# interaction-lab-uh/STROTSS-tensorflow

Measured on AMD Instinct MI355X. Metric: optimisation_steps_per_sec_1024px_pair, higher is better.
Workload: dtype f32; 1 GPU; 1024px content/style pair, 1024x1024 scale of the coarse-to-fine pyramid, 1024 samples x D=2179, VGG16 (seeded He-normal weights), RMSprop pixel update; scale_px=1024, samples=1024, parallelism=single GPU, tap_adjoint=deterministic (planned, sorted scatter)

## Files before the change

strotss-tensorflow_amd/csrc/image.hip:

```cpp
#include "internal.h"

namespace {

struct AxisTap { int lo, hi; float lerp; };
__device__ __forceinline__ AxisTap axis_tap(int i, float scale, int in_size) {
  const float src = __fsub_rn(__fmul_rn(__fadd_rn((float)i, 0.5f), scale), 0.5f);
  const float fl = floorf(src);
  AxisTap t;
  t.lo = max((int)fl, 0);
  t.hi = min((int)ceilf(src), in_size - 1);
  t.lerp = __fsub_rn(src, fl);
  return t;
}

template <int C>
__global__ __launch_bounds__(256) void resize_bilinear_kernel(const float* __restrict__ in, int ih, int iw,
                                                              int c_rt, float* __restrict__ out, int oh, int ow,
                                                              float sy, float sx, float alpha,
                                                              const float* __restrict__ add) {
  const int c = C ? C : c_rt;
  for (int oy = blockIdx.y; oy < oh; oy += gridDim.y) {
    const AxisTap ty = axis_tap(oy, sy, ih);
    const float* r0 = in + (size_t)ty.lo * iw * c;
    const float* r1 = in + (size_t)ty.hi * iw * c;
    const size_t orow = (size_t)oy * ow * c;
    for (int ox = blockIdx.x * 256 + threadIdx.x; ox < ow; ox += gridDim.x * 256) {
      const AxisTap tx = axis_tap(ox, sx, iw);
      const int a = tx.lo * c, b = tx.hi * c;
      const size_t o = orow + (size_t)ox * c;
#pragma unroll
      for (int ch = 0; ch < (C ? C : 1); ++ch)
        for (int cc = ch; cc < c; cc += (C ? C : 1)) {
          const float tl = r0[a + cc], tr = r0[b + cc], bl = r1[a + cc], br = r1[b + cc];
          const float top = tl + (tr - tl) * tx.lerp;
          const float bot = bl + (br - bl) * tx.lerp;
          float v = alpha * (top + (bot - top) * ty.lerp);
          if (add) v += add[o + cc];
          out[o + cc] = v;
        }
    }
  }
}

#define FOLD_TILE 32
#define FOLD_REGION 24
struct FoldLevels { int n; int h[STROTSS_MAX_TENSORS], w[STROTSS_MAX_TENSORS]; const float* v[STROTSS_MAX_TENSORS]; };
__device__ __forceinline__ float bilerp3(float tl, float tr, float bl, float br, float lx, float ly) {
  const float top = tl + (tr - tl) * lx;
  const float bot = bl + (br - bl) * lx;
  return 1.0f * (top + (bot - top) * ly);
}
__global__ __launch_bounds__(256) void fold_pyramid_kernel(FoldLevels p, float* __restrict__ img) {
  __shared__ float buf[2][FOLD_REGION * FOLD_REGION * 3];
  __shared__ int reg[STROTSS_MAX_TENSORS][4];
  const int t = threadIdx.x;
  if (t == 0) {
    int y0 = blockIdx.y * FOLD_TILE, y1 = min(y0 + FOLD_TILE, p.h[0]) - 1;
    int x0 = blockIdx.x * FOLD_TILE, x1 = min(x0 + FOLD_TILE, p.w[0]) - 1;
    reg[0][0] = y0; reg[0][1] = y1; reg[0][2] = x0; reg[0][3] = x1;
    for (int k = 1; k < p.n; ++k) {
      const float sy = (float)p.h[k] / (float)p.h[k - 1], sx = (float)p.w[k] / (float)p.w[k - 1];
      const int ny0 = axis_tap(y0, sy, p.h[k]).lo, ny1 = axis_tap(y1, sy, p.h[k]).hi;
      const int nx0 = axis_tap(x0, sx, p.w[k]).lo, nx1 = axis_tap(x1, sx, p.w[k]).hi;
      y0 = ny0; y1 = ny1; x0 = nx0; x1 = nx1;
      reg[k][0] = y0; reg[k][1] = y1; reg[k][2] = x0; reg[k][3] = x1;
    }
  }
  __syncthreads();
  {
    const int k = p.n - 1, y0 = reg[k][0], x0 = reg[k][2], rh = reg[k][1] - y0 + 1, rw = reg[k][3] - x0 + 1;
    float* dst = buf[k & 1];
    for (int e = t; e < rh * rw; e += 256) {
      const int ry = e / rw, rx = e - ry * rw;
      const float* s = p.v[k] + ((size_t)(y0 + ry) * p.w[k] + x0 + rx) * 3;
      dst[e * 3 + 0] = s[0]; dst[e * 3 + 1] = s[1]; dst[e * 3 + 2] = s[2];
    }
  }
  __syncthreads();
  for (int k = p.n - 2; k >= 0; --k) {
    const int y0 = reg[k][0], x0 = reg[k][2], rh = reg[k][1] - y0 + 1, rw = reg[k][3] - x0 + 1;
    const int cy0 = reg[k + 1][0], cx0 = reg[k + 1][2], cw = reg[k + 1][3] - cx0 + 1;
    const int ih = p.h[k + 1], iw = p.w[k + 1];
    const float sy = (float)ih / (float)p.h[k], sx = (float)iw / (float)p.w[k];
    const float* src = buf[(k + 1) & 1];
    float* dst = k == 0 ? nullptr : buf[k & 1];
    for (int e = t; e < rh * rw; e += 256) {
      const int ry = e / rw, rx = e - ry * rw;
      const int oy = y0 + ry, ox = x0 + rx;
      const AxisTap ty = axis_tap(oy, sy, ih), tx = axis_tap(ox, sx, iw);
      const float* r0 = src + (size_t)(ty.lo - cy0) * cw * 3;
      const float* r1 = src + (size_t)(ty.hi - cy0) * cw * 3;
      const int a = (tx.lo - cx0) * 3, b = (tx.hi - cx0) * 3;
      const size_t o = ((size_t)oy * p.w[k] + ox) * 3;
      const float* add = p.v[k] + o;
#pragma unroll
      for (int c = 0; c < 3; ++c) {
        float v = bilerp3(r0[a + c], r0[b + c], r1[a + c], r1[b + c], tx.lerp, ty.lerp);
        v += add[c];
        if (k == 0) img[o + c] = v; else dst[e * 3 + c] = v;
      }
    }
    __syncthreads();
  }
}

#define ADJ_MAX 8
__device__ __forceinline__ float adj_weight(int o, float scale, int in_size, int i) {
  const AxisTap t = axis_tap(o, scale, in_size);
  return (t.lo == i ? 1.0f - t.lerp : 0.f) + (t.hi == i ? t.lerp : 0.f);
}
struct AdjGlobal3 {
  const float* p; int ow;
  __device__ __forceinline__ const float* at(int oy, int ox) const { return p + ((size_t)oy * ow + ox) * 3; }
};
struct AdjRegion3 {
  const float* p; int y0, x0, rw;
  __device__ __forceinline__ const float* at(int oy, int ox) const { return p + ((oy - y0) * rw + (ox - x0)) * 3; }
};
__device__ __forceinline__ void adj_range(int i, float inv_scale, int out_size, int& o0, int& o1) {
  o0 = max(0, (int)floorf(((float)i - 0.5f) * inv_scale - 0.5f) - 1);
  o1 = min(out_size - 1, (int)ceilf(((float)i + 1.5f) * inv_scale - 0.5f) + 1);
}
template <class Src>
__device__ __forceinline__ void adjoint_pixel3(const Src& g, int oh, int ow, int ih, int iw, float sy, float sx, int iy,
                                               int ix, float (&acc)[3]) {
  int oy0, oy1, ox0, ox1;
  adj_range(iy, 1.0f / sy, oh, oy0, oy1);
  adj_range(ix, 1.0f / sx, ow, ox0, ox1);
  acc[0] = acc[1] = acc[2] = 0.f;
  if (ox1 - ox0 < ADJ_MAX) {
    float wx[ADJ_MAX];
#pragma unroll
    for (int q = 0; q < ADJ_MAX; ++q) wx[q] = (ox0 + q <= ox1) ? adj_weight(ox0 + q, sx, iw, ix) : 0.f;
    for (int oy = oy0; oy <= oy1; ++oy) {
      const float wy = adj_weight(oy, sy, ih, iy);
      if (wy == 0.f) continue;
      float row[3] = {0.f, 0.f, 0.f};
#pragma unroll
      for (int q = 0; q < ADJ_MAX; ++q)
        if (wx[q] != 0.f) {
          const float* p = g.at(oy, ox0 + q);
#pragma unroll
          for (int ch = 0; ch < 3; ++ch) row[ch] += wx[q] * p[ch];
        }
#pragma unroll
      for (int ch = 0; ch < 3; ++ch) acc[ch] += wy * row[ch];
    }
    return;
  }
  for (int oy = oy0; oy <= oy1; ++oy) {
    const float wy = adj_weight(oy, sy, ih, iy);
    if (wy == 0.f) continue;
    float row[3] = {0.f, 0.f, 0.f};
    for (int ox = ox0; ox <= ox1; ++ox) {
      const float w = adj_weight(ox, sx, iw, ix);
      if (w != 0.f) {
        const float* q = g.at(oy, ox);
#pragma unroll
        for (int ch = 0; ch < 3; ++ch) row[ch] += w * q[ch];
      }
    }
#pragma unroll
    for (int ch = 0; ch < 3; ++ch) acc[ch] += wy * row[ch];
  }
}

#define ADJ2_T2 8
#define ADJ2_REGION 32
__global__ __launch_bounds__(256) void resize_adjoint_pair_kernel(const float* __restrict__ g0, int h0, int w0,
                                                                  float* __restrict__ g1, int h1, int w1,
                                                                  float* __restrict__ g2, int h2, int w2) {
  __shared__ float mid[ADJ2_REGION * ADJ2_REGION * 3];
  const int t = threadIdx.x;
  const float sy1 = (float)h1 / (float)h0, sx1 = (float)w1 / (float)w0;
  const float sy2 = (float)h2 / (float)h1, sx2 = (float)w2 / (float)w1;
  const int ty0 = blockIdx.y * ADJ2_T2, ty1 = min(ty0 + ADJ2_T2, h2) - 1, tx0 = blockIdx.x * ADJ2_T2, tx1 = min(tx0 + ADJ2_T2, w2) - 1;
  const int oy0 = blockIdx.y * 2 * ADJ2_T2, oy1 = min(oy0 + 2 * ADJ2_T2, h1) - 1;
  const int ox0 = blockIdx.x * 2 * ADJ2_T2, ox1 = min(ox0 + 2 * ADJ2_T2, w1) - 1;
  const bool has2 = ty0 <= ty1 && tx0 <= tx1, own1 = oy0 <= oy1 && ox0 <= ox1;
  int ry0 = oy0, ry1 = oy1, rx0 = ox0, rx1 = ox1;
  if (has2) {
    int a, b, c, d;
    adj_range(ty0, 1.0f / sy2, h1, a, b); adj_range(ty1, 1.0f / sy2, h1, c, d);
    const int ny0 = a, ny1 = d;
    adj_range(tx0, 1.0f / sx2, w1, a, b); adj_range(tx1, 1.0f / sx2, w1, c, d);
    const int nx0 = a, nx1 = d;
    if (own1) { ry0 = min(ry0, ny0); ry1 = max(ry1, ny1); rx0 = min(rx0, nx0); rx1 = max(rx1, nx1); }
    else { ry0 = ny0; ry1 = ny1; rx0 = nx0; rx1 = nx1; }
  } else if (!own1) {
    return;
  }
  const int rh = ry1 - ry0 + 1, rw = rx1 - rx0 + 1;
  const AdjGlobal3 src0{g0, w0};
  for (int e = t; e < rh * rw; e += 256) {
    const int ry = e / rw, rx = e - ry * rw;
    const int iy = ry0 + ry, ix = rx0 + rx;
    float acc[3];
    adjoint_pixel3(src0, h0, w0, h1, w1, sy1, sx1, iy, ix, acc);
    mid[e * 3 + 0] = acc[0]; mid[e * 3 + 1] = acc[1]; mid[e * 3 + 2] = acc[2];
    if (own1 && iy >= oy0 && iy <= oy1 && ix >= ox0 && ix <= ox1) {
      float* o = g1 + ((size_t)iy * w1 + ix) * 3;
      o[0] = acc[0]; o[1] = acc[1]; o[2] = acc[2];
    }
  }
  __syncthreads();
  if (!has2) return;
  const AdjRegion3 src1{mid, ry0, rx0, rw};
  const int th = ty1 - ty0 + 1, tw = tx1 - tx0 + 1;
  for (int e = t; e < th * tw; e += 256) {
    const int iy = ty0 + e / tw, ix = tx0 + e % tw;
    float acc[3];
    adjoint_pixel3(src1, h1, w1, h2, w2, sy2, sx2, iy, ix, acc);
    float* o = g2 + ((size_t)iy * w2 + ix) * 3;
    o[0] = acc[0]; o[1] = acc[1]; o[2] = acc[2];
  }
}

template <int C>
__global__ __launch_bounds__(256) void resize_adjoint_kernel(const float* __restrict__ gout, int oh, int ow,
                                                             int c_rt, float* __restrict__ gin, int ih, int iw,
                                                             float sy, float sx) {
  const int c = C ? C : c_rt;
  const float isy = 1.0f / sy, isx = 1.0f / sx;
  for (int iy = blockIdx.y; iy < ih; iy += gridDim.y) {
    const int oy0 = max(0, (int)floorf(((float)iy - 0.5f) * isy - 0.5f) - 1);
    const int oy1 = min(oh - 1, (int)ceilf(((float)iy + 1.5f) * isy - 0.5f) + 1);
    for (int ix = blockIdx.x * 256 + threadIdx.x; ix < iw; ix += gridDim.x * 256) {
      const int ox0 = max(0, (int)floorf(((float)ix - 0.5f) * isx - 0.5f) - 1);
      const int ox1 = min(ow - 1, (int)ceilf(((float)ix + 1.5f) * isx - 0.5f) + 1);
      float acc[C ? C : 4];
#pragma unroll
      for (int ch = 0; ch < (C ? C : 4); ++ch) acc[ch] = 0.f;
      if (C && ox1 - ox0 < ADJ_MAX) {
        float wx[ADJ_MAX];
#pragma unroll
        for (int q = 0; q < ADJ_MAX; ++q) wx[q] = (ox0 + q <= ox1) ? adj_weight(ox0 + q, sx, iw, ix) : 0.f;
        for (int oy = oy0; oy <= oy1; ++oy) {
          const float wy = adj_weight(oy, sy, ih, iy);
          if (wy == 0.f) continue;
          const float* g = gout + ((size_t)oy * ow + ox0) * c;
          float row[C ? C : 1];
#pragma unroll
          for (int ch = 0; ch < C; ++ch) row[ch] = 0.f;
#pragma unroll
          for (int q = 0; q < ADJ_MAX; ++q)
            if (wx[q] != 0.f) {
#pragma unroll
              for (int ch = 0; ch < C; ++ch) row[ch] += wx[q] * g[q * c + ch];
            }
#pragma unroll
          for (int ch = 0; ch < C; ++ch) acc[ch] += wy * row[ch];
        }
#pragma unroll
        for (int ch = 0; ch < C; ++ch) gin[((size_t)iy * iw + ix) * c + ch] = acc[ch];
      } else {
        for (int ch0 = 0; ch0 < c; ch0 += 4) {
          const int nc = min(4, c - ch0);
          float a4[4] = {0.f, 0.f, 0.f, 0.f};
          for (int oy = oy0; oy <= oy1; ++oy) {
            const float wy = adj_weight(oy, sy, ih, iy);
            if (wy == 0.f) continue;
            float row[4] = {0.f, 0.f, 0.f, 0.f};
            for (int ox = ox0; ox <= ox1; ++ox) {
              const float w = adj_weight(ox, sx, iw, ix);
              if (w != 0.f)
                for (int ch = 0; ch < nc; ++ch) row[ch] += w * gout[((size_t)oy * ow + ox) * c + ch0 + ch];
            }
            for (int ch = 0; ch < nc; ++ch) a4[ch] += wy * row[ch];
          }
          for (int ch = 0; ch < nc; ++ch) gin[((size_t)iy * iw + ix) * c + ch0 + ch] = a4[ch];
        }
      }
    }
  }
}

struct SampleTap { int ia, ib, ic, id; float wa, wb, wc, wd; };

__device__ __forceinline__ SampleTap sample_tap(const strotss_maps_t& m, int k, float gx, float gy,
                                                int bilinear) {
  for (int q = 0; q < m.n_div[k]; ++q) {
    gx = __fdiv_rn(gx, m.div[q]);
    gy = __fdiv_rn(gy, m.div[q]);
  }
  const int h = m.h[k], w = m.w[k];
  SampleTap t;
  if (bilinear) {
    const float gxf = floorf(gx), gyf = floorf(gy);
    const float dx = gx - gxf, dy = gy - gyf;
    t.wa = (1.f - dx) * (1.f - dy);
    t.wb = (1.f - dx) * dy;
    t.wc = dx * (1.f - dy);
    t.wd = dx * dy;
    const int x0 = (int)fminf(fmaxf(gxf, 0.f), (float)(h - 1));
    const int y0 = (int)fminf(fmaxf(gyf, 0.f), (float)(w - 1));
    int x1 = min(x0 + 1, h - 1);
    const int y1 = min(y0 + 1, w - 1);
    int xa = x0;
    if (m.rows[k] > 0) {
      const int ra = x0 - m.row0[k], rb = x1 - m.row0[k];
      xa = min(max(ra, 0), m.rows[k] - 1);
      x1 = min(max(rb, 0), m.rows[k] - 1);
      if (m.window_drop & (int)(ra != xa)) { t.wa = 0.f; t.wb = 0.f; }
      if (m.window_drop & (int)(rb != x1)) { t.wc = 0.f; t.wd = 0.f; }
    }
    t.ia = xa * w + y0; t.ib = xa * w + y1; t.ic = x1 * w + y0; t.id = x1 * w + y1;
  } else {
    int xi = (int)fminf(fmaxf(gx, 0.f), (float)(h - 1));
    const int yi = (int)fminf(fmaxf(gy, 0.f), (float)(w - 1));
    if (m.rows[k] > 0) xi = min(max(xi - m.row0[k], 0), m.rows[k] - 1);
    t.ia = t.ib = t.ic = t.id = xi * w + yi;
    t.wa = 1.f; t.wb = t.wc = t.wd = 0.f;
  }
  return t;
}

__device__ __forceinline__ void gather_row(const strotss_maps_t& m, const float* __restrict__ idx, int s, int bilinear,
                                           float* __restrict__ out, int ld, int dtotal) {
  if (m.sample_range && (s < m.sample_range[0] || s >= m.sample_range[1])) return;
  const float gx = idx[2 * s], gy = idx[2 * s + 1];
  float* o = out + (size_t)s * ld;
  const int wave = __builtin_amdgcn_readfirstlane((int)threadIdx.x >> 6), lane = threadIdx.x & 63;
  int off = 0, chunk = 0;
  for (int k = 0; k < m.n_maps; ++k) {
    const int c = m.c[k], nchunk = (c + 63) >> 6;
    int q0 = (wave - chunk) & 3;
    if (q0 < nchunk) {
      const SampleTap t = sample_tap(m, k, gx, gy, bilinear);
      const float* src = m.map[k];
      if (bilinear) {
        const float* pa = src + (size_t)t.ia * c; const float* pb = src + (size_t)t.ib * c;
        const float* pc = src + (size_t)t.ic * c; const float* pd = src + (size_t)t.id * c;
        for (int q = q0; q < nchunk; q += 4) {
          const int ch = q * 64 + lane;
          if (ch < c) o[off + ch] = pa[ch] * t.wa + pb[ch] * t.wb + pc[ch] * t.wc + pd[ch] * t.wd;
        }
      } else {
        const float* pa = src + (size_t)t.ia * c;
        for (int q = q0; q < nchunk; q += 4) {
          const int ch = q * 64 + lane;
          if (ch < c) o[off + ch] = pa[ch];
        }
      }
    }
    off += c;
    chunk += nchunk;
  }
  for (int ch = dtotal + threadIdx.x; ch < ld; ch += 256) o[ch] = 0.f;
}
__global__ __launch_bounds__(256) void hypercol_gather_kernel(strotss_maps_t m, const float* __restrict__ idx,
                                                              int bilinear, float* __restrict__ out, int ld,
                                                              int dtotal) {
  gather_row(m, idx, blockIdx.x, bilinear, out, ld, dtotal);
}
__device__ __forceinline__ void gather2_body(const strotss_maps_t& ma, const strotss_maps_t& mb,
                                             const float* __restrict__ idx, int n, int bilinear, float* __restrict__ out_a,
                                             float* __restrict__ out_b, int ld, int dtotal_a, int dtotal_b,
                                             float* __restrict__ zero, int zero_rows, const int b) {
  if (b < n) {
    gather_row(ma, idx, b, bilinear, out_a, ld, dtotal_a);
    if (zero) {
      const int r1 = b == n - 1 ? zero_rows : min(b + 1, zero_rows);
      for (int r = b; r < r1; ++r)
        for (int ch = threadIdx.x; ch < ld; ch += 256) zero[(size_t)r * ld + ch] = 0.f;
    }
  } else {
    gather_row(mb, idx, b - n, bilinear, out_b, ld, dtotal_b);
  }
}
__global__ __launch_bounds__(256) void hypercol_gather2_kernel(strotss_maps_t ma, strotss_maps_t mb,
                                                               const float* __restrict__ idx, int n, int bilinear,
                                                               float* __restrict__ out_a, float* __restrict__ out_b, int ld,
                                                               int dtotal_a, int dtotal_b, float* __restrict__ zero,
                                                               int zero_rows) {
  gather2_body(ma, mb, idx, n, bilinear, out_a, out_b, ld, dtotal_a, dtotal_b, zero, zero_rows, (int)blockIdx.x);
}
__global__ __launch_bounds__(256) void hypercol_gather2_cw_kernel(strotss_maps_t ma, strotss_maps_t mb, strotss_maps_t mw,
                                                                  const float* __restrict__ idx, int n, int bilinear,
                                                                  float* __restrict__ out_a, float* __restrict__ out_b, int ld,
                                                                  int dtotal_a, int dtotal_b, float* __restrict__ zero,
                                                                  int zero_rows, float* __restrict__ wout, int wrows) {
  const int b = blockIdx.x;
  gather2_body(ma, mb, idx, n, bilinear, out_a, out_b, ld, dtotal_a, dtotal_b, zero, zero_rows, b);
  if (b < n) {
    gather_row(mw, idx, b, bilinear, wout, 1, 1);
    if (b == n - 1)
      for (int r = n + (int)threadIdx.x; r < wrows; r += 256) wout[r] = 0.f;
  }
}
#define SCATTER_DENSE_MAX_PIX 64
__device__ __forceinline__ void scatter_dense_block(const strotss_maps_t& m, const float* __restrict__ idx, int n,
                                                    const float* __restrict__ gfeat, int ld, bool masked, int k, int off, int b) {
  __shared__ int li[1024];
  __shared__ float lw[1024];
  __shared__ int cnts[4];
  __shared__ float red[4][64];
  const int tid = threadIdx.x, lane = tid & 63, wave = tid >> 6;
  const int c = m.c[k], nchunk = (c + 63) >> 6;
  const int p = b / nchunk, q = b - p * nchunk;
  const int s0 = m.sample_range ? m.sample_range[0] : 0, s1 = m.sample_range ? min(n, m.sample_range[1]) : n;
  const int ch = q * 64 + lane;
  const bool in = ch < c;
  const float* g = gfeat + off + (in ? ch : c - 1);
  float acc = 0.f;
  for (int base = s0; base < s1; base += 1024) {
    float w4[4];
    int cnt = 0;
#pragma unroll
    for (int u = 0; u < 4; ++u) {
      const int s = base + 4 * tid + u;
      float w = 0.f;
      if (s < s1) {
        const SampleTap t = sample_tap(m, k, idx[2 * s], idx[2 * s + 1], 1);
        w = (t.ia == p ? t.wa : 0.f) + (t.ib == p ? t.wb : 0.f) + (t.ic == p ? t.wc : 0.f) + (t.id == p ? t.wd : 0.f);
      }
      w4[u] = w;
      cnt += w != 0.f;
    }
    int incl = cnt;
#pragma unroll
    for (int o = 1; o < 64; o <<= 1) {
      const int up = __shfl_up(incl, o, 64);
      if (lane >= o) incl += up;
    }
    __syncthreads();
    if (lane == 63) cnts[wave] = incl;
    __syncthreads();
    int at = incl - cnt, total = 0;
#pragma unroll
    for (int wv = 0; wv < 4; ++wv) {
      at += wv < wave ? cnts[wv] : 0;
      total += cnts[wv];
    }
#pragma unroll
    for (int u = 0; u < 4; ++u)
      if (w4[u] != 0.f) { li[at] = base + 4 * tid + u; lw[at] = w4[u]; ++at; }
    __syncthreads();
    int e = wave;
    for (; e + 12 < total; e += 16) {
      float v[4];
#pragma unroll
      for (int u = 0; u < 4; ++u) v[u] = g[(size_t)li[e + 4 * u] * ld];
#pragma unroll
      for (int u = 0; u < 4; ++u) acc += lw[e + 4 * u] * v[u];
    }
    for (; e < total; e += 4) acc += lw[e] * g[(size_t)li[e] * ld];
  }
  red[wave][lane] = acc;
  __syncthreads();
  if (wave == 0 && in) {
    const float tot = (red[0][lane] + red[1][lane]) + (red[2][lane] + red[3][lane]);
    const size_t o = (size_t)p * c + ch;
    if (tot != 0.f && (!masked || m.map[k][o] > 0.f)) m.gmap[k][o] += tot;
  }
}
__global__ __launch_bounds__(256) void hypercol_scatter_kernel(strotss_maps_t m, const float* __restrict__ idx,
                                                               const float* __restrict__ gfeat, int ld,
                                                               int relu_mask_from, int map_begin,
                                                               int map_end, int n, unsigned dense_mask, int dense_blocks) {
  if ((int)blockIdx.x < dense_blocks) {
    int b = (int)blockIdx.x, off = 0;
    for (int k = 0; k < map_end; ++k) {
      if ((dense_mask >> k) & 1u) {
        const int nb = (m.rows[k] > 0 ? m.rows[k] : m.h[k]) * m.w[k] * ((m.c[k] + 63) >> 6);
        if (b < nb) { scatter_dense_block(m, idx, n, gfeat, ld, k >= relu_mask_from, k, off, b); return; }
        b -= nb;
      }
      off += m.c[k];
    }
    return;
  }
  const int s = (int)blockIdx.x - dense_blocks;
  if (m.sample_range && (s < m.sample_range[0] || s >= m.sample_range[1])) return;
  const float gx = idx[2 * s], gy = idx[2 * s + 1];
  const float* g = gfeat + (size_t)s * ld;
  const int wave = __builtin_amdgcn_readfirstlane((int)threadIdx.x >> 6), lane = threadIdx.x & 63;
  int off = 0, chunk = 0;
  for (int k = 0; k < map_end; ++k) {
    const int c = m.c[k], nchunk = (c + 63) >> 6;
    const int q0 = (wave - chunk) & 3;
    chunk += nchunk;
    if (k < map_begin || q0 >= nchunk || ((dense_mask >> k) & 1u)) { off += c; continue; }
    const SampleTap t = sample_tap(m, k, gx, gy, 1);
    const float* act = m.map[k];
    float* dst = m.gmap[k];
    const bool masked = k >= relu_mask_from;
    const int ii[4] = {t.ia, t.ib, t.ic, t.id};
    const float ww[4] = {t.wa, t.wb, t.wc, t.wd};
    for (int q = q0; q < nchunk; q += 4) {
      const int ch = q * 64 + lane;
      const bool in = ch < c;
      const int chc = in ? ch : c - 1;
      const float gv = in ? g[off + chc] : 0.f;
#pragma unroll
      for (int tq = 0; tq < 4; ++tq) {
        const float v = ww[tq] * gv;
        const size_t o = (size_t)ii[tq] * c + chc;
        if (v != 0.f && (!masked || act[o] > 0.f)) atomicAdd(&dst[o], v);
      }
    }
    off += c;
  }
}

#define PLAN_E 4096
struct PlanView {
  int* nseg; int* seg_start; int* pix; int* smp; float* w;
  __host__ __device__ static size_t ints_per_map() { return 2 + (PLAN_E + 1) + 3 * (size_t)PLAN_E + 1; }
  __host__ __device__ PlanView(void* base, int k) {
    int* b = reinterpret_cast<int*>(base) + (size_t)k * ints_per_map();
    nseg = b; seg_start = b + 2; pix = seg_start + PLAN_E + 1; smp = pix + PLAN_E; w = reinterpret_cast<float*>(smp + PLAN_E);
  }
};
__global__ __launch_bounds__(1024) void scatter_plan_kernel(strotss_maps_t m, const float* __restrict__ idx, int n,
                                                            void* __restrict__ plan) {
  __shared__ unsigned long long key[PLAN_E];
  __shared__ int wsum[16];
  const int k = blockIdx.x, t = threadIdx.x;
  const unsigned long long INVALID = ~0ull;
  const int s_begin = m.sample_range ? m.sample_range[0] : 0, s_end = m.sample_range ? min(n, m.sample_range[1]) : n;
  for (int e = t; e < PLAN_E; e += 1024) {
    const int s = e >> 2, q = e & 3;
    unsigned long long kk = INVALID;
    if (s >= s_begin && s < s_end) {
      const SampleTap tp = sample_tap(m, k, idx[2 * s], idx[2 * s + 1], 1);
      const int ii = q == 0 ? tp.ia : q == 1 ? tp.ib : q == 2 ? tp.ic : tp.id;
      const float ww = q == 0 ? tp.wa : q == 1 ? tp.wb : q == 2 ? tp.wc : tp.wd;
      if (ww != 0.f) kk = ((unsigned long long)(unsigned)ii << 12) | (unsigned)e;
    }
    key[e] = kk;
  }
  __syncthreads();
  for (int size = 2; size <= PLAN_E; size <<= 1)
    for (int stride = size >> 1; stride > 0; stride >>= 1) {
      for (int p = t; p < PLAN_E / 2; p += 1024) {
        const int lo = 2 * p - (p & (stride - 1));
        const int hi = lo + stride;
        const bool up = (lo & size) == 0;
        const unsigned long long a = key[lo], b = key[hi];
        if ((a > b) == up) { key[lo] = b; key[hi] = a; }
      }
      __syncthreads();
    }
  PlanView pv(plan, k);
  int head[4], cnt = 0, valid = 0;
#pragma unroll
  for (int i = 0; i < 4; ++i) {
    const int p = 4 * t + i;
    const unsigned long long a = key[p];
    const bool ok = a != INVALID;
    head[i] = ok && (p == 0 || (key[p - 1] >> 12) != (a >> 12));
    cnt += head[i]; valid += ok;
  }
  int incl = cnt, vincl = valid;
#pragma unroll
  for (int o = 1; o < 64; o <<= 1) {
    const int u = __shfl_up(incl, o, 64), v = __shfl_up(vincl, o, 64);
    if ((t & 63) >= o) { incl += u; vincl += v; }
  }
  if ((t & 63) == 63) { wsum[t >> 6] = incl; }
  __syncthreads();
  int base = incl - cnt;
  for (int wv = 0; wv < (t >> 6); ++wv) base += wsum[wv];
  int total = 0;
#pragma unroll
  for (int wv = 0; wv < 16; ++wv) total += wsum[wv];
  __syncthreads();
  if ((t & 63) == 63) wsum[t >> 6] = vincl;
  __syncthreads();
  int nvalid = 0;
#pragma unroll
  for (int wv = 0; wv < 16; ++wv) nvalid += wsum[wv];
#pragma unroll
  for (int i = 0; i < 4; ++i) {
    const int p = 4 * t + i;
    const unsigned long long a = key[p];
    if (a == INVALID) continue;
    const int e = (int)(a & 4095u), s = e >> 2, q = e & 3;
    const SampleTap tp = sample_tap(m, k, idx[2 * s], idx[2 * s + 1], 1);
    pv.pix[p] = (int)(a >> 12);
    pv.smp[p] = s;
    pv.w[p] = q == 0 ? tp.wa : q == 1 ? tp.wb : q == 2 ? tp.wc : tp.wd;
    if (head[i]) pv.seg_start[base++] = p;
  }
  if (t == 0) { pv.nseg[0] = total; pv.seg_start[total] = nvalid; }
}
__global__ __launch_bounds__(256) void scatter_sorted_kernel(strotss_maps_t m, int k, int off, const void* __restrict__ plan,
                                                             const float* __restrict__ gfeat, int ld, int masked) {
  PlanView pv(const_cast<void*>(plan), k);
  const int sg = blockIdx.x;
  if (sg >= pv.nseg[0]) return;
  const int p0 = pv.seg_start[sg], p1 = pv.seg_start[sg + 1];
  const int c = m.c[k];
  const size_t pixel = (size_t)pv.pix[p0] * c;
  const float* act = m.map[k];
  float* dst = m.gmap[k];
  for (int ch = threadIdx.x; ch < c; ch += 256) {
    if (masked && !(act[pixel + ch] > 0.f)) continue;
    float acc = 0.f;
    for (int p = p0; p < p1; ++p) acc += pv.w[p] * gfeat[(size_t)pv.smp[p] * ld + off + ch];
    dst[pixel + ch] += acc;
  }
}

__global__ __launch_bounds__(256) void rmsprop_kernel(strotss_tensors_t t, float lr, float rho, float eps) {
  const int k = blockIdx.y;
  float* var = t.var[k];
  float* rms = t.rms[k];
  const float* g = t.grad[k];
  const int64_t n = t.numel[k];
  const float omr = 1.0f - rho;
  for (int64_t e = (int64_t)blockIdx.x * 256 + threadIdx.x; e < n; e += (int64_t)gridDim.x * 256) {
    const float gv = g[e];
    const float r = rho * rms[e] + omr * (gv * gv);
    rms[e] = r;
    var[e] = var[e] - lr * gv / (sqrtf(r) + eps);
  }
}

__global__ __launch_bounds__(256) void minmax_partial_kernel(const float* __restrict__ x, int64_t n,
                                                             float* __restrict__ ws) {
  __shared__ float red[4];
  float mn = INFINITY, mx = -INFINITY;
  for (int64_t e = (int64_t)blockIdx.x * 256 + threadIdx.x; e < n; e += (int64_t)gridDim.x * 256) {
    const float v = fminf(fmaxf(x[e], 0.f), 1.f);
    mn = fminf(mn, v);
    mx = fmaxf(mx, v);
  }
  mn = block_min_256(mn, red);
  mx = block_max_256(mx, red);
  if (threadIdx.x == 0) { ws[blockIdx.x] = mn; ws[1024 + blockIdx.x] = mx; }
}
__global__ __launch_bounds__(256) void postprocess_kernel(const float* __restrict__ x, int64_t n,
                                                          const float* __restrict__ ws, int nparts,
                                                          uint8_t* __restrict__ out) {
  __shared__ float red[4];
  float mn = INFINITY, mx = -INFINITY;
  for (int i = threadIdx.x; i < nparts; i += 256) { mn = fminf(mn, ws[i]); mx = fmaxf(mx, ws[1024 + i]); }
  mn = block_min_256(mn, red);
  mx = block_max_256(mx, red);
  const float range = mx - mn;
  for (int64_t e = (int64_t)blockIdx.x * 256 + threadIdx.x; e < n; e += (int64_t)gridDim.x * 256) {
    float v = fminf(fmaxf(x[e], 0.f), 1.f);
    v = (v - mn) / range;
    out[e] = (uint8_t)(v * 255.0f);
  }
}

int maps_ok(const strotss_maps_t* m) {
  if (!m || m->n_maps <= 0 || m->n_maps > STROTSS_MAX_MAPS) return 0;
  for (int k = 0; k < m->n_maps; ++k) {
    if (m->h[k] <= 0 || m->w[k] <= 0 || m->c[k] <= 0 || !m->map[k]) return 0;
    if (m->n_div[k] < 0 || m->n_div[k] > STROTSS_MAX_DIVS) return 0;
    if (m->rows[k] < 0 || m->row0[k] < 0 || m->row0[k] + m->rows[k] > m->h[k]) return 0;
  }
  return 1;
}

}

extern "C" {

int strotss_abi_version(void) { return 8; }
const char* strotss_build_info(void) { return "libstrotss_hip gfx950 fp32-mfma " __DATE__ " " __TIME__; }

int strotss_resize_bilinear(const float* in, int ih, int iw, int c, float* out, int oh, int ow, float alpha,
                            const float* add, void* stream) {
  ST_CHECK_ARG(in && out && ih > 0 && iw > 0 && oh > 0 && ow > 0 && c > 0, STROTSS_EINVAL);
  const float sy = (float)ih / (float)oh, sx = (float)iw / (float)ow;
  const dim3 grid((unsigned)cdiv(ow, 256), (unsigned)min(oh, 32768));
  if (c == 3)
    hipLaunchKernelGGL(resize_bilinear_kernel<3>, grid, dim3(256), 0, (hipStream_t)stream, in, ih, iw, c, out, oh, ow, sy, sx,
                       alpha, add);
  else if (c == 1)
    hipLaunchKernelGGL(resize_bilinear_kernel<1>, grid, dim3(256), 0, (hipStream_t)stream, in, ih, iw, c, out, oh, ow, sy, sx,
                       alpha, add);
  else
    hipLaunchKernelGGL(resize_bilinear_kernel<0>, grid, dim3(256), 0, (hipStream_t)stream, in, ih, iw, c, out, oh, ow, sy, sx,
                       alpha, add);
  ST_LAUNCH_RET();
}

int strotss_fold_pyramid(const strotss_pyramid_t* pyr, float* img, void* stream) {
  ST_CHECK_ARG(pyr && img && pyr->n_levels >= 2 && pyr->n_levels <= STROTSS_MAX_TENSORS, STROTSS_EINVAL);
  FoldLevels p;
  p.n = pyr->n_levels;
  for (int k = 0; k < p.n; ++k) {
    ST_CHECK_ARG(pyr->var[k] && pyr->h[k] > 0 && pyr->w[k] > 0, STROTSS_EINVAL);
    p.h[k] = pyr->h[k]; p.w[k] = pyr->w[k]; p.v[k] = pyr->var[k];
  }
  int sy = FOLD_TILE, sx = FOLD_TILE;
  for (int k = 1; k < p.n; ++k) {
    ST_CHECK_ARG(p.h[k] <= p.h[k - 1] && p.w[k] <= p.w[k - 1], STROTSS_ERANGE);
    sy = min(p.h[k], (int)((long long)sy * p.h[k] / p.h[k - 1]) + 3);
    sx = min(p.w[k], (int)((long long)sx * p.w[k] / p.w[k - 1]) + 3);
    ST_CHECK_ARG(sy <= FOLD_REGION && sx <= FOLD_REGION, STROTSS_ERANGE);
  }
  hipLaunchKernelGGL(fold_pyramid_kernel, dim3((unsigned)cdiv(p.w[0], FOLD_TILE), (unsigned)cdiv(p.h[0], FOLD_TILE)), dim3(256),
                     0, (hipStream_t)stream, p, img);
  ST_LAUNCH_RET();
}

static bool adjoint_pair_ok(int a, int b) { return b >= 1 && a >= 2 * b - 1 && a <= 2 * b + 1; }

int strotss_fold_pyramid_adjoint(const strotss_pyramid_t* g, void* stream) {
  ST_CHECK_ARG(g && g->n_levels >= 2 && g->n_levels <= STROTSS_MAX_TENSORS, STROTSS_EINVAL);
  for (int k = 0; k < g->n_levels; ++k) ST_CHECK_ARG(g->var[k] && g->h[k] > 0 && g->w[k] > 0, STROTSS_EINVAL);
  int k = 0;
  while (k + 1 < g->n_levels) {
    const bool pair = k + 2 < g->n_levels && adjoint_pair_ok(g->h[k], g->h[k + 1]) && adjoint_pair_ok(g->w[k], g->w[k + 1]) &&
                      adjoint_pair_ok(g->h[k + 1], g->h[k + 2]) && adjoint_pair_ok(g->w[k + 1], g->w[k + 2]);
    if (pair) {
      const unsigned gx = (unsigned)max(cdiv(g->w[k + 2], ADJ2_T2), cdiv(g->w[k + 1], 2 * ADJ2_T2));
      const unsigned gy = (unsigned)max(cdiv(g->h[k + 2], ADJ2_T2), cdiv(g->h[k + 1], 2 * ADJ2_T2));
      hipLaunchKernelGGL(resize_adjoint_pair_kernel, dim3(gx, gy), dim3(256), 0, (hipStream_t)stream,
                         (const float*)g->var[k], g->h[k], g->w[k], const_cast<float*>(g->var[k + 1]), g->h[k + 1], g->w[k + 1],
                         const_cast<float*>(g->var[k + 2]), g->h[k + 2], g->w[k + 2]);
      k += 2;
    } else {
      const int rc = strotss_resize_bilinear_adjoint(g->var[k], g->h[k], g->w[k], 3, const_cast<float*>(g->var[k + 1]),
                                                     g->h[k + 1], g->w[k + 1], stream);
      if (rc != 0) return rc;
      k += 1;
    }
  }
  ST_LAUNCH_RET();
}

int strotss_resize_bilinear_adjoint(const float* gout, int oh, int ow, int c, float* gin, int ih, int iw,
                                    void* stream) {
  ST_CHECK_ARG(gout && gin && ih > 0 && iw > 0 && oh > 0 && ow > 0 && c > 0, STROTSS_EINVAL);
  const float sy = (float)ih / (float)oh, sx = (float)iw / (float)ow;
  const dim3 grid((unsigned)cdiv(iw, 256), (unsigned)min(ih, 32768));
  if (c == 3)
    hipLaunchKernelGGL(resize_adjoint_kernel<3>, grid, dim3(256), 0, (hipStream_t)stream, gout, oh, ow, c, gin, ih, iw, sy, sx);
  else if (c == 1)
    hipLaunchKernelGGL(resize_adjoint_kernel<1>, grid, dim3(256), 0, (hipStream_t)stream, gout, oh, ow, c, gin, ih, iw, sy, sx);
  else
    hipLaunchKernelGGL(resize_adjoint_kernel<0>, grid, dim3(256), 0, (hipStream_t)stream, gout, oh, ow, c, gin, ih, iw, sy, sx);
  ST_LAUNCH_RET();
}

int strotss_hypercol_gather(const strotss_maps_t* maps, const float* idx, int n, int bilinear, float* out,
                            int ld, void* stream) {
  ST_CHECK_ARG(maps_ok(maps) && idx && out && n > 0, STROTSS_EINVAL);
  int d = 0;
  for (int k = 0; k < maps->n_maps; ++k) d += maps->c[k];
  ST_CHECK_ARG(ld >= d, STROTSS_EINVAL);
  strotss_maps_t m = *maps;
  m.window_drop = 0;
  hipLaunchKernelGGL(hypercol_gather_kernel, dim3(n), dim3(256), 0, (hipStream_t)stream, m, idx, bilinear,
                     out, ld, d);
  ST_LAUNCH_RET();
}

int strotss_hypercol_gather2(const strotss_maps_t* maps_a, const strotss_maps_t* maps_b, const float* idx, int n,
                             int bilinear, float* out_a, float* out_b, int ld, float* zero, int zero_rows, void* stream) {
  ST_CHECK_ARG(maps_ok(maps_a) && maps_ok(maps_b) && idx && out_a && out_b && n > 0, STROTSS_EINVAL);
  ST_CHECK_ARG(!zero || zero_rows > 0, STROTSS_EINVAL);
  int da = 0, db = 0;
  for (int k = 0; k < maps_a->n_maps; ++k) da += maps_a->c[k];
  for (int k = 0; k < maps_b->n_maps; ++k) db += maps_b->c[k];
  ST_CHECK_ARG(ld >= da && ld >= db, STROTSS_EINVAL);
  strotss_maps_t a = *maps_a, b = *maps_b;
  a.window_drop = b.window_drop = 0;
  hipLaunchKernelGGL(hypercol_gather2_kernel, dim3(2 * n), dim3(256), 0, (hipStream_t)stream, a, b, idx, n, bilinear, out_a,
                     out_b, ld, da, db, zero, zero_rows);
  ST_LAUNCH_RET();
}

int strotss_hypercol_gather2_cw(const strotss_maps_t* maps_a, const strotss_maps_t* maps_b, const strotss_maps_t* maps_w,
                                const float* idx, int n, int bilinear, float* out_a, float* out_b, int ld, float* zero,
                                int zero_rows, float* weight_out, int weight_rows, void* stream) {
  ST_CHECK_ARG(maps_ok(maps_a) && maps_ok(maps_b) && maps_ok(maps_w) && idx && out_a && out_b && weight_out && n > 0,
               STROTSS_EINVAL);
  ST_CHECK_ARG(maps_w->n_maps == 1 && maps_w->c[0] == 1 && maps_w->rows[0] == 0 && weight_rows >= n, STROTSS_EINVAL);
  ST_CHECK_ARG(!zero || zero_rows > 0, STROTSS_EINVAL);
  int da = 0, db = 0;
  for (int k = 0; k < maps_a->n_maps; ++k) da += maps_a->c[k];
  for (int k = 0; k < maps_b->n_maps; ++k) db += maps_b->c[k];
  ST_CHECK_ARG(ld >= da && ld >= db, STROTSS_EINVAL);
  strotss_maps_t a = *maps_a, b = *maps_b, wm = *maps_w;
  a.window_drop = b.window_drop = wm.window_drop = 0;
  wm.sample_range = nullptr;
  hipLaunchKernelGGL(hypercol_gather2_cw_kernel, dim3(2 * n), dim3(256), 0, (hipStream_t)stream, a, b, wm, idx, n, bilinear,
                     out_a, out_b, ld, da, db, zero, zero_rows, weight_out, weight_rows);
  ST_LAUNCH_RET();
}

int strotss_hypercol_scatter(const strotss_maps_t* maps, const float* idx, int n, const float* gfeat, int ld,
                             int relu_mask_from, int map_begin, int map_end, void* stream) {
  ST_CHECK_ARG(maps_ok(maps) && idx && gfeat && n > 0, STROTSS_EINVAL);
  ST_CHECK_ARG(map_begin >= 0 && map_begin < map_end && map_end <= maps->n_maps, STROTSS_ERANGE);
  int d = 0;
  for (int k = 0; k < maps->n_maps; ++k) {
    if (k >= map_begin && k < map_end) ST_CHECK_ARG(maps->gmap[k] != nullptr, STROTSS_EINVAL);
    d += maps->c[k];
  }
  ST_CHECK_ARG(ld >= d, STROTSS_EINVAL);
  static const int dense_pix = [] {
    const char* e = getenv("STROTSS_SCATTER_DENSE");
    const int v = e ? atoi(e) : 1;
    return v == 1 ? SCATTER_DENSE_MAX_PIX : v;
  }();
  unsigned dense_mask = 0;
  int dense_blocks = 0;
  for (int k = map_begin; k < map_end; ++k) {
    const int pix = (maps->rows[k] > 0 ? maps->rows[k] : maps->h[k]) * maps->w[k];
    if (pix <= dense_pix) { dense_mask |= 1u << k; dense_blocks += pix * ((maps->c[k] + 63) / 64); }
  }
  hipLaunchKernelGGL(hypercol_scatter_kernel, dim3(n + dense_blocks), dim3(256), 0, (hipStream_t)stream, *maps, idx, gfeat,
                     ld, relu_mask_from, map_begin, map_end, n, dense_mask, dense_blocks);
  ST_LAUNCH_RET();
}

size_t strotss_hypercol_scatter_plan_bytes(int n_maps) {
  return n_maps > 0 ? (size_t)n_maps * PlanView::ints_per_map() * sizeof(int) : 0;
}

int strotss_hypercol_scatter_plan(const strotss_maps_t* maps, const float* idx, int n, void* plan, size_t plan_bytes,
                                  void* stream) {
  ST_CHECK_ARG(maps_ok(maps) && idx && plan && n > 0, STROTSS_EINVAL);
  ST_CHECK_ARG(4 * n <= PLAN_E, STROTSS_ERANGE);
  ST_CHECK_ARG(plan_bytes >= strotss_hypercol_scatter_plan_bytes(maps->n_maps), STROTSS_EINVAL);
  for (int k = 0; k < maps->n_maps; ++k) {
    const long long px = (long long)(maps->rows[k] > 0 ? maps->rows[k] : maps->h[k]) * maps->w[k];
    ST_CHECK_ARG(px < (1ll << 31), STROTSS_ERANGE);
  }
  hipLaunchKernelGGL(scatter_plan_kernel, dim3(maps->n_maps), dim3(1024), 0, (hipStream_t)stream, *maps, idx, n, plan);
  ST_LAUNCH_RET();
}

int strotss_hypercol_scatter_sorted(const strotss_maps_t* maps, const void* plan, int n, const float* gfeat, int ld,
                                    int relu_mask_from, int map_begin, int map_end, void* stream) {
  ST_CHECK_ARG(maps_ok(maps) && plan && gfeat && n > 0 && 4 * n <= PLAN_E, STROTSS_EINVAL);
  ST_CHECK_ARG(map_begin >= 0 && map_begin < map_end && map_end <= maps->n_maps, STROTSS_ERANGE);
  int off = 0;
  for (int k = 0; k < map_end; ++k) {
    if (k >= map_begin) {
      ST_CHECK_ARG(maps->gmap[k] != nullptr && off + maps->c[k] <= ld, STROTSS_EINVAL);
      hipLaunchKernelGGL(scatter_sorted_kernel, dim3(4 * n), dim3(256), 0, (hipStream_t)stream, *maps, k, off, plan, gfeat,
                         ld, k >= relu_mask_from ? 1 : 0);
    }
    off += maps->c[k];
  }
  ST_LAUNCH_RET();
}

int strotss_rmsprop_step(const strotss_tensors_t* t, float lr, float rho, float eps, void* stream) {
  ST_CHECK_ARG(t && t->n_tensors > 0 && t->n_tensors <= STROTSS_MAX_TENSORS, STROTSS_ERANGE);
  int64_t mx = 0;
  for (int k = 0; k < t->n_tensors; ++k) {
    ST_CHECK_ARG(t->var[k] && t->rms[k] && t->grad[k] && t->numel[k] > 0, STROTSS_EINVAL);
    mx = t->numel[k] > mx ? t->numel[k] : mx;
  }
  dim3 grid((unsigned)((mx + 255) / 256 > 2048 ? 2048 : (mx + 255) / 256), t->n_tensors);
  hipLaunchKernelGGL(rmsprop_kernel, grid, dim3(256), 0, (hipStream_t)stream, *t, lr, rho, eps);
  ST_LAUNCH_RET();
}

int strotss_postprocess(const float* img, int64_t numel, uint8_t* out, float* workspace, void* stream) {
  ST_CHECK_ARG(img && out && workspace && numel > 0, STROTSS_EINVAL);
  const int nparts = (int)((numel + 255) / 256 > 1024 ? 1024 : (numel + 255) / 256);
  hipLaunchKernelGGL(minmax_partial_kernel, dim3(nparts), dim3(256), 0, (hipStream_t)stream, img, numel,
                     workspace);
  hipLaunchKernelGGL(postprocess_kernel, dim3(nparts), dim3(256), 0, (hipStream_t)stream, img, numel,
                     workspace, nparts, out);
  ST_LAUNCH_RET();
}

}
```

strotss-tensorflow_amd/csrc/sort_match.h:

```cpp
#pragma once
#include "common.h"

namespace {

constexpr int SORT_T = 1024;

__device__ __forceinline__ unsigned long long ordered_pack(float v, int idx) {
  unsigned b = __float_as_uint(v);
  if (b == 0x80000000u) b = 0u;
  const unsigned key = (b & 0x80000000u) ? ~b : (b | 0x80000000u);
  return ((unsigned long long)key << 32) | (unsigned)idx;
}
__device__ __forceinline__ float ordered_value(unsigned long long c) {
  const unsigned key = (unsigned)(c >> 32);
  return __uint_as_float((key & 0x80000000u) ? (key & 0x7FFFFFFFu) : ~key);
}

template <int SIDES>
__device__ __forceinline__ void bitonic_sort_1024(unsigned long long (&v)[SIDES], unsigned long long* buf0,
                                                  unsigned long long* buf1, int S) {
  const int tid = threadIdx.x;
  int cross = 0;
#pragma unroll
  for (int k = 2; k <= SORT_T; k <<= 1) {
#pragma unroll
    for (int j = k >> 1; j > 0; j >>= 1) {
      unsigned long long* const buf = (cross & 1) ? buf1 : buf0;
      if (j >= 64) ++cross;
      if (k > S) continue;
      unsigned long long pv[SIDES];
      if (j < 64) {
#pragma unroll
        for (int s = 0; s < SIDES; ++s)
          pv[s] = ((unsigned long long)__shfl_xor((unsigned)(v[s] >> 32), j, 64) << 32) | __shfl_xor((unsigned)v[s], j, 64);
      } else {
#pragma unroll
        for (int s = 0; s < SIDES; ++s) buf[s * SORT_T + tid] = v[s];
        __syncthreads();
#pragma unroll
        for (int s = 0; s < SIDES; ++s) pv[s] = buf[s * SORT_T + (tid ^ j)];
      }
      const bool keep_low = ((tid & j) == 0) == ((tid & k) == 0);
#pragma unroll
      for (int s = 0; s < SIDES; ++s) v[s] = (v[s] < pv[s]) == keep_low ? v[s] : pv[s];
    }
  }
}

struct SquaredCost {
  static __device__ __forceinline__ void pair(float len, float diff, float& g, float& w) {
    g += len * diff;
    w += len * diff * diff;
  }
};
struct AbsoluteCost {
  static __device__ __forceinline__ void pair(float len, float diff, float& g, float& w) {
    g += diff > 0.f ? len : (diff < 0.f ? -len : 0.f);
    w += len * fabsf(diff);
  }
};

struct QuantileMatch {
  float coef;
  int row;
  float cost;
};

template <class Cost>
__device__ __forceinline__ QuantileMatch quantile_match(unsigned long long va, unsigned long long vb, int n, int ns,
                                                        float* sb) {
  const int tid = threadIdx.x;
  if (tid < ns) sb[tid] = ordered_value(vb);
  __syncthreads();
  QuantileMatch m = {0.f, 0, 0.f};
  if (tid < n) {
    const float a = ordered_value(va);
    const int lo = tid * ns, hi = lo + ns;
    float g = 0.f, w = 0.f;
    for (int j = lo / n; j < ns && j * n < hi; ++j) {
      const float len = (float)(min(hi, (j + 1) * n) - max(lo, j * n));
      const float diff = a - sb[j];
      Cost::pair(len, diff, g, w);
    }
    const float inv = (float)(1.0 / ((double)n * ns));
    m.coef = g * inv;
    m.row = (int)(unsigned)(va & 0xFFFFFFFFull);
    m.cost = w * inv;
  }
  return m;
}

__device__ __forceinline__ double block_sum_f64_1024(double v, double* red) {
  const int tid = threadIdx.x;
  v = wave_sum(v);
  if ((tid & 63) == 0) red[tid >> 6] = v;
  __syncthreads();
  double s = 0.0;
  if (tid == 0) {
#pragma unroll
    for (int i = 0; i < SORT_T / 64; ++i) s += red[i];
  }
  return s;
}

}
```

Measured before the change: 217.5 steps/s.

## Sort scatter-plan keys in registers with wave shuffles instead of LDS bitonic

```diff
diff --git a/strotss-tensorflow_amd/csrc/image.hip b/strotss-tensorflow_amd/csrc/image.hip
--- a/strotss-tensorflow_amd/csrc/image.hip
+++ b/strotss-tensorflow_amd/csrc/image.hip
@@ -1,4 +1,5 @@
 #include "internal.h"
+#include "sort_match.h"
 
 namespace {
 
@@ -514,76 +515,68 @@
 };
 __global__ __launch_bounds__(1024) void scatter_plan_kernel(strotss_maps_t m, const float* __restrict__ idx, int n,
                                                             void* __restrict__ plan) {
-  __shared__ unsigned long long key[PLAN_E];
-  __shared__ int wsum[16];
-  const int k = blockIdx.x, t = threadIdx.x;
+  __shared__ unsigned long long buf[2 * PLAN_E];
+  const int k = blockIdx.x, t = threadIdx.x, lane = t & 63, wave = t >> 6;
   const unsigned long long INVALID = ~0ull;
   const int s_begin = m.sample_range ? m.sample_range[0] : 0, s_end = m.sample_range ? min(n, m.sample_range[1]) : n;
-  for (int e = t; e < PLAN_E; e += 1024) {
-    const int s = e >> 2, q = e & 3;
-    unsigned long long kk = INVALID;
-    if (s >= s_begin && s < s_end) {
-      const SampleTap tp = sample_tap(m, k, idx[2 * s], idx[2 * s + 1], 1);
-      const int ii = q == 0 ? tp.ia : q == 1 ? tp.ib : q == 2 ? tp.ic : tp.id;
-      const float ww = q == 0 ? tp.wa : q == 1 ? tp.wb : q == 2 ? tp.wc : tp.wd;
-      if (ww != 0.f) kk = ((unsigned long long)(unsigned)ii << 12) | (unsigned)e;
-    }
-    key[e] = kk;
-  }
+  unsigned long long v[4] = {INVALID, INVALID, INVALID, INVALID};
+  float ww[4] = {0.f, 0.f, 0.f, 0.f};
+  if (t >= s_begin && t < s_end) {
+    const SampleTap tp = sample_tap(m, k, idx[2 * t], idx[2 * t + 1], 1);
+    const int ii[4] = {tp.ia, tp.ib, tp.ic, tp.id};
+    ww[0] = tp.wa; ww[1] = tp.wb; ww[2] = tp.wc; ww[3] = tp.wd;
+#pragma unroll
+    for (int q = 0; q < 4; ++q)
+      if (ww[q] != 0.f) v[q] = ((unsigned long long)(unsigned)ii[q] << 12) | (unsigned)(4 * t + q);
+  }
+  bitonic_sort_owned<4>(v, buf, buf + PLAN_E);
+  float* const wtab = reinterpret_cast<float*>(buf);
+  unsigned* const edge = reinterpret_cast<unsigned*>(wtab + PLAN_E);
+  int* const wsum = reinterpret_cast<int*>(edge + 16);
+  unsigned px[4];
+#pragma unroll
+  for (int i = 0; i < 4; ++i) px[i] = (unsigned)(v[i] >> 12);
+  *reinterpret_cast<float4*>(wtab + 4 * t) = make_float4(ww[0], ww[1], ww[2], ww[3]);
+  if (lane == 63) edge[wave] = px[3];
   __syncthreads();
-  for (int size = 2; size <= PLAN_E; size <<= 1)
-    for (int stride = size >> 1; stride > 0; stride >>= 1) {
-      for (int p = t; p < PLAN_E / 2; p += 1024) {
-        const int lo = 2 * p - (p & (stride - 1));
-        const int hi = lo + stride;
-        const bool up = (lo & size) == 0;
-        const unsigned long long a = key[lo], b = key[hi];
-        if ((a > b) == up) { key[lo] = b; key[hi] = a; }
-      }
-      __syncthreads();
-    }
+  unsigned prev = __shfl_up(px[3], 1, 64);
+  if (lane == 0 && wave > 0) prev = edge[wave - 1];
+  int head[4], cnt = 0, valid = 0;
+#pragma unroll
+  for (int i = 0; i < 4; ++i) {
+    const bool ok = v[i] != INVALID;
+    head[i] = ok && (4 * t + i == 0 || (i ? px[i - 1] : prev) != px[i]);
+    cnt += head[i]; valid += ok;
+  }
+  const int both = cnt | (valid << 16);
+  int incl = both;
+#pragma unroll
+  for (int o = 1; o < 64; o <<= 1) {
+    const int u = __shfl_up(incl, o, 64);
+    if (lane >= o) incl += u;
+  }
+  if (lane == 63) wsum[wave] = incl;
+  __syncthreads();
+  int base = incl - both, total = 0;
+#pragma unroll
+  for (int wv = 0; wv < 16; ++wv) { const int c = wsum[wv]; base += wv < wave ? c : 0; total += c; }
+  base &= 0xFFFF;
+  const int nseg = total & 0xFFFF, nvalid = total >> 16;
   PlanView pv(plan, k);
-  int head[4], cnt = 0, valid = 0;
 #pragma unroll
   for (int i = 0; i < 4; ++i) {
-    const int p = 4 * t + i;
-    const unsigned long long a = key[p];
-    const bool ok = a != INVALID;
-    head[i] = ok && (p == 0 || (key[p - 1] >> 12) != (a >> 12));
-    cnt += head[i]; valid += ok;
-  }
-  int incl = cnt, vincl = valid;
-#pragma unroll
-  for (int o = 1; o < 64; o <<= 1) {
-    const int u = __shfl_up(incl, o, 64), v = __shfl_up(vincl, o, 64);
-    if ((t & 63) >= o) { incl += u; vincl += v; }
-  }
-  if ((t & 63) == 63) { wsum[t >> 6] = incl; }
-  __syncthreads();
-  int base = incl - cnt;
-  for (int wv = 0; wv < (t >> 6); ++wv) base += wsum[wv];
-  int total = 0;
-#pragma unroll
-  for (int wv = 0; wv < 16; ++wv) total += wsum[wv];
-  __syncthreads();
-  if ((t & 63) == 63) wsum[t >> 6] = vincl;
-  __syncthreads();
-  int nvalid = 0;
-#pragma unroll
-  for (int wv = 0; wv < 16; ++wv) nvalid += wsum[wv];
-#pragma unroll
-  for (int i = 0; i < 4; ++i) {
-    const int p = 4 * t + i;
-    const unsigned long long a = key[p];
-    if (a == INVALID) continue;
-    const int e = (int)(a & 4095u), s = e >> 2, q = e & 3;
-    const SampleTap tp = sample_tap(m, k, idx[2 * s], idx[2 * s + 1], 1);
-    pv.pix[p] = (int)(a >> 12);
-    pv.smp[p] = s;
-    pv.w[p] = q == 0 ? tp.wa : q == 1 ? tp.wb : q == 2 ? tp.wc : tp.wd;
+    const int p = 4 * t + i, e = (int)(v[i] & 4095u);
+    if (v[i] == INVALID) continue;
+    pv.pix[p] = (int)px[i]; pv.smp[p] = e >> 2; pv.w[p] = wtab[e];
     if (head[i]) pv.seg_start[base++] = p;
   }
-  if (t == 0) { pv.nseg[0] = total; pv.seg_start[total] = nvalid; }
+  if (t == 0) { pv.nseg[0] = nseg; pv.seg_start[nseg] = nvalid; }
+}
+__global__ __launch_bounds__(1024) void scatter_plan_lds_kernel(strotss_maps_t, const float*, int, void*);
+void launch_scatter_plan(const strotss_maps_t& m, const float* idx, int n, void* plan, hipStream_t s) {
+  static const bool lds = [] { const char* e = getenv("STROTSS_SCATTER_PLAN_LDS"); return e && atoi(e) != 0; }();
+  if (lds) hipLaunchKernelGGL(scatter_plan_lds_kernel, dim3(m.n_maps), dim3(1024), 0, s, m, idx, n, plan);
+  else hipLaunchKernelGGL(scatter_plan_kernel, dim3(m.n_maps), dim3(1024), 0, s, m, idx, n, plan);
 }
 __global__ __launch_bounds__(256) void scatter_sorted_kernel(strotss_maps_t m, int k, int off, const void* __restrict__ plan,
                                                              const float* __restrict__ gfeat, int ld, int masked) {
@@ -827,7 +820,7 @@
     const long long px = (long long)(maps->rows[k] > 0 ? maps->rows[k] : maps->h[k]) * maps->w[k];
     ST_CHECK_ARG(px < (1ll << 31), STROTSS_ERANGE);
   }
-  hipLaunchKernelGGL(scatter_plan_kernel, dim3(maps->n_maps), dim3(1024), 0, (hipStream_t)stream, *maps, idx, n, plan);
+  launch_scatter_plan(*maps, idx, n, plan, (hipStream_t)stream);
   ST_LAUNCH_RET();
 }
 
@@ -870,3 +863,81 @@
 }
 
 }
+
+namespace {
+
+__global__ __launch_bounds__(1024) void scatter_plan_lds_kernel(strotss_maps_t m, const float* __restrict__ idx, int n,
+                                                                void* __restrict__ plan) {
+  __shared__ unsigned long long key[PLAN_E];
+  __shared__ int wsum[16];
+  const int k = blockIdx.x, t = threadIdx.x;
+  const unsigned long long INVALID = ~0ull;
+  const int s_begin = m.sample_range ? m.sample_range[0] : 0, s_end = m.sample_range ? min(n, m.sample_range[1]) : n;
+  for (int e = t; e < PLAN_E; e += 1024) {
+    const int s = e >> 2, q = e & 3;
+    unsigned long long kk = INVALID;
+    if (s >= s_begin && s < s_end) {
+      const SampleTap tp = sample_tap(m, k, idx[2 * s], idx[2 * s + 1], 1);
+      const int ii = q == 0 ? tp.ia : q == 1 ? tp.ib : q == 2 ? tp.ic : tp.id;
+      const float ww = q == 0 ? tp.wa : q == 1 ? tp.wb : q == 2 ? tp.wc : tp.wd;
+      if (ww != 0.f) kk = ((unsigned long long)(unsigned)ii << 12) | (unsigned)e;
+    }
+    key[e] = kk;
+  }
+  __syncthreads();
+  for (int size = 2; size <= PLAN_E; size <<= 1)
+    for (int stride = size >> 1; stride > 0; stride >>= 1) {
+      for (int p = t; p < PLAN_E / 2; p += 1024) {
+        const int lo = 2 * p - (p & (stride - 1));
+        const int hi = lo + stride;
+        const bool up = (lo & size) == 0;
+        const unsigned long long a = key[lo], b = key[hi];
+        if ((a > b) == up) { key[lo] = b; key[hi] = a; }
+      }
+      __syncthreads();
+    }
+  PlanView pv(plan, k);
+  int head[4], cnt = 0, valid = 0;
+#pragma unroll
+  for (int i = 0; i < 4; ++i) {
+    const int p = 4 * t + i;
+    const unsigned long long a = key[p];
+    const bool ok = a != INVALID;
+    head[i] = ok && (p == 0 || (key[p - 1] >> 12) != (a >> 12));
+    cnt += head[i]; valid += ok;
+  }
+  int incl = cnt, vincl = valid;
+#pragma unroll
+  for (int o = 1; o < 64; o <<= 1) {
+    const int u = __shfl_up(incl, o, 64), v = __shfl_up(vincl, o, 64);
+    if ((t & 63) >= o) { incl += u; vincl += v; }
+  }
+  if ((t & 63) == 63) { wsum[t >> 6] = incl; }
+  __syncthreads();
+  int base = incl - cnt;
+  for (int wv = 0; wv < (t >> 6); ++wv) base += wsum[wv];
+  int total = 0;
+#pragma unroll
+  for (int wv = 0; wv < 16; ++wv) total += wsum[wv];
+  __syncthreads();
+  if ((t & 63) == 63) wsum[t >> 6] = vincl;
+  __syncthreads();
+  int nvalid = 0;
+#pragma unroll
+  for (int wv = 0; wv < 16; ++wv) nvalid += wsum[wv];
+#pragma unroll
+  for (int i = 0; i < 4; ++i) {
+    const int p = 4 * t + i;
+    const unsigned long long a = key[p];
+    if (a == INVALID) continue;
+    const int e = (int)(a & 4095u), s = e >> 2, q = e & 3;
+    const SampleTap tp = sample_tap(m, k, idx[2 * s], idx[2 * s + 1], 1);
+    pv.pix[p] = (int)(a >> 12);
+    pv.smp[p] = s;
+    pv.w[p] = q == 0 ? tp.wa : q == 1 ? tp.wb : q == 2 ? tp.wc : tp.wd;
+    if (head[i]) pv.seg_start[base++] = p;
+  }
+  if (t == 0) { pv.nseg[0] = total; pv.seg_start[total] = nvalid; }
+}
+
+}
diff --git a/strotss-tensorflow_amd/csrc/sort_match.h b/strotss-tensorflow_amd/csrc/sort_match.h
--- a/strotss-tensorflow_amd/csrc/sort_match.h
+++ b/strotss-tensorflow_amd/csrc/sort_match.h
@@ -43,6 +43,50 @@
       const bool keep_low = ((tid & j) == 0) == ((tid & k) == 0);
 #pragma unroll
       for (int s = 0; s < SIDES; ++s) v[s] = (v[s] < pv[s]) == keep_low ? v[s] : pv[s];
+    }
+  }
+}
+
+template <int R>
+__device__ __forceinline__ void bitonic_sort_owned(unsigned long long (&v)[R], unsigned long long* buf0,
+                                                   unsigned long long* buf1) {
+  static_assert(R >= 1 && (R & (R - 1)) == 0, "keys per thread: a power of two");
+  const int tid = threadIdx.x;
+  int cross = 0;
+#pragma unroll
+  for (int k = 2; k <= R * SORT_T; k <<= 1) {
+#pragma unroll
+    for (int j = k >> 1; j > 0; j >>= 1) {
+      if (j < R) {
+#pragma unroll
+        for (int r = 0; r < R; ++r) {
+          if (r & j) continue;
+          const bool up = ((R * tid + r) & k) == 0;
+          const unsigned long long a = v[r], b = v[r | j];
+          const bool swap = (a > b) == up;
+          v[r] = swap ? b : a;
+          v[r | j] = swap ? a : b;
+        }
+        continue;
+      }
+      const int jt = j / R;
+      unsigned long long pv[R];
+      if (jt < 64) {
+#pragma unroll
+        for (int r = 0; r < R; ++r)
+          pv[r] = ((unsigned long long)__shfl_xor((unsigned)(v[r] >> 32), jt, 64) << 32) | __shfl_xor((unsigned)v[r], jt, 64);
+      } else {
+        unsigned long long* const buf = (cross & 1) ? buf1 : buf0;
+        ++cross;
+#pragma unroll
+        for (int r = 0; r < R; ++r) buf[r * SORT_T + tid] = v[r];
+        __syncthreads();
+#pragma unroll
+        for (int r = 0; r < R; ++r) pv[r] = buf[r * SORT_T + (tid ^ jt)];
+      }
+      const bool keep_low = ((tid & jt) == 0) == (((R * tid) & k) == 0);
+#pragma unroll
+      for (int r = 0; r < R; ++r) v[r] = (v[r] < pv[r]) == keep_low ? v[r] : pv[r];
     }
   }
 }
```

After: 218.6 steps/s (median of 6 runs). Within noise of the previous version (+0.5%).
